# givemeone1astkiss/RNA-MPNN

Hardware: AMD Instinct MI355X
Metric: nucleotides/sec (forward), k=30 RNA graphs (higher is better)
Workload: dtype bf16; 1 GPU; C2: batch=256 RNAs, n~U[100,140], k=30, default 10-layer RNAMPNN, P=T; max_len=140, weights=closed-form deterministic init (3,536,900 params), parallelism=dp1

## Files before the change

### rna-mpnn_amd/csrc/kernels_bf16.hip

```cpp
#include "kernels_bf16.h"
#include <cstdio>
#include <cstdlib>
#include <type_traits>

#include "bf16_dev.h"
#include "graph_norm_dev.h"

__global__ void k_convert_rows_bf16(const float* __restrict__ src, int ld_src, int rows, int cols, int cols_pad,
                                    bf16_t* __restrict__ dst) {
    int id = blockIdx.x * blockDim.x + threadIdx.x;
    if (id >= rows * cols_pad) return;
    int r = id / cols_pad, c = id - r * cols_pad;
    dst[id] = c < cols ? f2bf(src[(size_t)r * ld_src + c]) : (bf16_t)0;
}
void launch_convert_rows_bf16(const float* src, int ld_src, int rows, int cols, int cols_pad, bf16_t* dst, hipStream_t s) {
    int total = rows * cols_pad;
    hipLaunchKernelGGL(k_convert_rows_bf16, dim3((total + 255) / 256), dim3(256), 0, s, src, ld_src, rows, cols, cols_pad, dst);
}

__global__ void k_build_mlp_image(const float* __restrict__ wc, int ld_wc, const float* __restrict__ w2, int ld_w2,
                                  const float* __restrict__ b2, int out_perm, bf16_t* __restrict__ img, float* __restrict__ b2p) {
    int id = blockIdx.x * blockDim.x + threadIdx.x;
    if (!w2) {
        if (id < 2 * 32 * 64 * 8) {
// ... 525 lines not shown
#undef RN_FRAG
}

static int num_cus() { return rn_num_cus(); }

void launch_mpnn_bf16(const PackInfo& pk, int k, bool do_edge, bool do_msg, const int* nbr, bf16_t* e,
                      const bf16_t* p_e, const bf16_t* q_e, const bf16_t* p_m, const bf16_t* q_m, MpnnWB we, MpnnWB wm,
                      float* agg, float* msg_out, bool edge1, const float* h_res, int reverse, hipStream_t s) {
    if (resmpnn_covers(k, edge1, msg_out != nullptr)) {
        launch_resmpnn_bf16(pk, k, do_edge, do_msg, nbr, e, p_e, q_e, p_m, q_m, we, wm, agg, h_res, reverse, s);
        return;
    }
    const int npb = k > 16 ? 1 : 32 / k;
    const int max_blocks = (pk.Nmax + npb - 1) / npb;
    int grid = (max_blocks + RN_MPNN_WAVES - 1) / RN_MPNN_WAVES;
    if (grid >= 8) grid = (grid + 7) & ~7;
    if (grid > num_cus()) grid = num_cus();
    if (grid < 1) grid = 1;
    size_t lds = RN_MPNN_LDS;
    NodeTabs tab{p_e, q_e, p_m, q_m, h_res};
    const bool smallk = k <= 16, mo = msg_out != nullptr;
#define RN_LAUNCH(E, M, S, O, E1)                                                                              \
    do {                                                                                                       \
        static DevAttr attr;                                                                                   \
        ensure_dyn_lds((const void*)k_mpnn_bf16<E, M, S, O, E1>, RN_MPNN_LDS, attr);                           \
        hipLaunchKernelGGL((k_mpnn_bf16<E, M, S, O, E1>), dim3(grid), dim3(RN_MPNN_WAVES * 64), lds, s, pk, k, nbr, e, tab, we, wm, agg, msg_out); \
    } while (0)
    if (do_edge && do_msg && edge1) { if (smallk) RN_LAUNCH(true, true, true, false, true); else RN_LAUNCH(true, true, false, false, true); }
    else if (do_edge && edge1)      { if (smallk) RN_LAUNCH(true, false, true, false, true); else RN_LAUNCH(true, false, false, false, true); }
    else if (do_edge && do_msg) { if (smallk) RN_LAUNCH(true, true, true, false, false); else RN_LAUNCH(true, true, false, false, false); }
    else if (do_edge)      { if (smallk) RN_LAUNCH(true, false, true, false, false); else RN_LAUNCH(true, false, false, false, false); }
    else if (mo)           { if (smallk) RN_LAUNCH(false, true, true, true, false); else RN_LAUNCH(false, true, false, true, false); }
    else                   { if (smallk) RN_LAUNCH(false, true, true, false, false); else RN_LAUNCH(false, true, false, false, false); }
#undef RN_LAUNCH
}

#define RN_EE_FENCE() __builtin_amdgcn_sched_barrier(0)
#ifndef EE_WAVES
#define EE_WAVES 8
#endif
template <bool SMALLK>
__global__ void __launch_bounds__(EE_WAVES * 64, EE_WAVES / 2) k_edge_embed_bf16(PackInfo pk, int k, const float* __restrict__ geomh,
        const int* __restrict__ nbr, const bf16_t* __restrict__ img_g, const float* __restrict__ b0,
        const float* __restrict__ b1p, bf16_t* __restrict__ e) {
    extern __shared__ __attribute__((aligned(16))) unsigned char smem[];
    u32x4* img = reinterpret_cast<u32x4*>(smem);
    constexpr int NFRAG = 4 * EMB_KS + 32;
    const int tid = threadIdx.x;
    float* lds_b = reinterpret_cast<float*>(smem + (size_t)NFRAG * 1024);
    if (tid < 128) lds_b[tid] = kGA * b0[tid];
    else if (tid < 256) lds_b[tid] = b1p[tid - 128];
    {
        constexpr int NT = EE_WAVES * 64, PER = (NFRAG * 64 + NT - 1) / NT;
        u32x4 t[PER];
#pragma unroll
        for (int i = 0; i < PER; ++i) t[i] = reinterpret_cast<const u32x4*>(img_g)[min(tid + i * NT, NFRAG * 64 - 1)];
#pragma unroll
        for (int i = 0; i < PER; ++i) if (tid + i * NT < NFRAG * 64) img[tid + i * NT] = t[i];
    }
    __syncthreads();
    const int ntot = pk.cu[pk.B];
    const int npb = SMALLK ? 32 / k : 1;
    const int nblocks = (ntot + npb - 1) / npb;
    const int wave = tid >> 6, lane = tid & 63, r = lane & 31, h = lane >> 5;
    const int q0 = SMALLK ? r / k : 0;
    const bool slot_ok = SMALLK ? q0 < npb : r < k;
    const int last_idx = ntot * k - 1;
    const int stride = gridDim.x * EE_WAVES;

    auto load_j = [&](int b) -> int {
        const int i = b * npb * k + r;
        const int jr = nbr[min(max(i, 0), max(last_idx, 0))];
        return (b < nblocks && slot_ok && b * npb + q0 < ntot) ? jr : -1;
    };
    f32x4 nrec[7];
    auto load_rec = [&](int j) {
        const f32x4* src = reinterpret_cast<const f32x4*>(geomh + (size_t)(j >= 0 ? j : 0) * RN_GEOMH + 32 * h);
#pragma unroll
        for (int v = 0; v < 7; ++v) nrec[v] = src[v];
    };
    int blk = blockIdx.x * EE_WAVES + wave;
    if (blk >= nblocks) return;
    int j_cur = load_j(blk), j_nxt = load_j(blk + stride);
    load_rec(j_cur);

    for (; blk < nblocks; blk += stride) {
        const int cnode = SMALLK ? min(blk * npb + q0, ntot - 1) : __builtin_amdgcn_readfirstlane(blk);
        const float* __restrict__ gc = geomh + (size_t)cnode * RN_GEOMH;
        auto catom = [&](int a, int d) { return a < 4 ? gc[3 * a + d] : gc[32 + 3 * (a - 4) + d]; };
        auto cbond = [&](int a, int d) { return a < 3 ? gc[12 + 3 * a + d] : gc[32 + 12 + 3 * (a - 3) + d]; };
        auto cnorm = [&](int a, int d) { return a < 2 ? gc[21 + 3 * a + d] : gc[32 + 21 + 3 * (a - 2) + d]; };
        float nl[28];
#pragma unroll
        for (int v = 0; v < 7; ++v) { nl[4 * v] = nrec[v][0]; nl[4 * v + 1] = nrec[v][1]; nl[4 * v + 2] = nrec[v][2]; nl[4 * v + 3] = nrec[v][3]; }
        float ft[EMB_SLOTS];
#pragma unroll
        for (int a = 0; a < 7; ++a) {
            const float ax = catom(a, 0), ay = catom(a, 1), az = catom(a, 2);
#pragma unroll
            for (int bl = 0; bl < 4; ++bl) {
                const float dx = nl[3 * bl] - ax, dy = nl[3 * bl + 1] - ay, dz = nl[3 * bl + 2] - az;
                ft[4 * a + bl] = __builtin_amdgcn_sqrtf(fmaf(dz, dz, fmaf(dy, dy, fmaf(dx, dx, kSEPS))));
            }
        }
#pragma unroll
        for (int a = 0; a < 5; ++a) {
            const float ax = cbond(a, 0), ay = cbond(a, 1), az = cbond(a, 2);
#pragma unroll
            for (int bl = 0; bl < 3; ++bl) ft[28 + 3 * a + bl] = fmaf(az, nl[12 + 3 * bl + 2], fmaf(ay, nl[12 + 3 * bl + 1], ax * nl[12 + 3 * bl]));
        }
#pragma unroll
        for (int a = 0; a < 4; ++a) {
            const float ax = cnorm(a, 0), ay = cnorm(a, 1), az = cnorm(a, 2);
#pragma unroll
            for (int bl = 0; bl < 2; ++bl) ft[43 + 2 * a + bl] = fmaf(az, nl[21 + 3 * bl + 2], fmaf(ay, nl[21 + 3 * bl + 1], ax * nl[21 + 3 * bl]));
        }
#pragma unroll
        for (int p = 51; p < EMB_SLOTS; ++p) ft[p] = 0.f;
        u32x4 xf[EMB_KS];
#pragma unroll
        for (int s = 0; s < EMB_KS; ++s)
#pragma unroll
            for (int t = 0; t < 4; ++t) xf[s][t] = p_pack2(ft[8 * s + 2 * t], ft[8 * s + 2 * t + 1]);
        RN_EE_FENCE();
        const unsigned vmask = j_cur >= 0 ? 0xffffffffu : 0u;
        load_rec(j_nxt);
        j_cur = j_nxt;
        j_nxt = load_j(blk + 2 * stride);
        RN_EE_FENCE();

        u32x4 hb[8];
#pragma unroll
        for (int mb = 0; mb < 4; ++mb) {
            f32x16 acc = init_vec16(lds_b + 32 * mb + 16 * h);
#pragma unroll
            for (int s = 0; s < EMB_KS; ++s) acc = mfma32h(img[(mb * EMB_KS + s) * 64 + lane], xf[s], acc);
#pragma unroll
            for (int t = 0; t < 4; ++t) {
                const f16x4 x = cvt_h4(acc[2 * t], acc[2 * t + 1], acc[8 + 2 * t], acc[8 + 2 * t + 1]);
                const f16x4 g = x * phi4s(x);
                hb[2 * mb][t] = __builtin_bit_cast(unsigned, lo2(g));
                hb[2 * mb + 1][t] = __builtin_bit_cast(unsigned, hi2(g));
            }
            RN_EE_FENCE();
        }
        u32x4* ewp = efrag_ptr(e, blk, lane);
#pragma unroll
        for (int ob = 0; ob < 4; ++ob) {
            f32x16 acc = init_vec16(lds_b + 128 + 32 * ob + 16 * h);
#pragma unroll
            for (int ks = 0; ks < 8; ++ks) acc = mfma32h(img[(4 * EMB_KS + ob * 8 + ks) * 64 + lane], hb[ks], acc);
#pragma unroll
            for (int sp = 0; sp < 2; ++sp) {
                u32x4 nw;
#pragma unroll
                for (int t = 0; t < 4; t += 2) {
                    const f16x4 xq = cvt_h4(acc[8 * sp + 2 * t], acc[8 * sp + 2 * t + 1], acc[8 * sp + 2 * t + 2], acc[8 * sp + 2 * t + 3]);
                    const f16x4 gq4 = xq * phi4s(xq);
                    nw[t] = __builtin_bit_cast(unsigned, lo2(gq4)) & vmask;
                    nw[t + 1] = __builtin_bit_cast(unsigned, hi2(gq4)) & vmask;
                }
                ewp[64 * (2 * ob + sp)] = nw;
            }
            RN_EE_FENCE();
        }
    }
}

void launch_edge_embed_bf16(const PackInfo& pk, int k, const float* geomh, const int* nbr, const bf16_t* img,
                            const float* b0, const float* b1p, bf16_t* e, hipStream_t s) {
    const int npb = k > 16 ? 1 : 32 / k;
    const int max_blocks = (pk.Nmax + npb - 1) / npb;
    int grid = (max_blocks + EE_WAVES - 1) / EE_WAVES;
    if (grid > 2 * num_cus()) grid = 2 * num_cus();
    if (grid < 1) grid = 1;
    size_t lds = (size_t)(4 * EMB_KS + 32) * 1024 + 1024;
    if (k > 16) hipLaunchKernelGGL(k_edge_embed_bf16<false>, dim3(grid), dim3(EE_WAVES * 64), lds, s, pk, k, geomh, nbr, img, b0, b1p, e);
    else hipLaunchKernelGGL(k_edge_embed_bf16<true>, dim3(grid), dim3(EE_WAVES * 64), lds, s, pk, k, geomh, nbr, img, b0, b1p, e);
}

#define GB_LD 72
__global__ void __launch_bounds__(256) k_gemm_bf16(const int* __restrict__ ntot_p, const float* __restrict__ X, int ldx, int K1,
        const float* __restrict__ X2, int ldx2, int K2, const bf16_t* __restrict__ W, const float* __restrict__ bias,
        int N, int act, const float* __restrict__ res, int ldres, float* __restrict__ Y, int ldy) {
    __shared__ __attribute__((aligned(16))) bf16_t As[128 * GB_LD];
    __shared__ __attribute__((aligned(16))) bf16_t Bs[128 * GB_LD];
    const int ntot = *ntot_p;
    const int row0 = blockIdx.x * 128;
    if (row0 >= ntot) return;
    const int col0 = blockIdx.y * 128;
    const int K = K1 + K2;
    const int tid = threadIdx.x, lane = tid & 63, wave = tid >> 6;
    const int r = lane & 31, h = lane >> 5;
    const int wr = wave >> 1, wc = wave & 1;
    const int srow = tid >> 1, shalf = tid & 1;

    f32x16 acc[2][2];
#pragma unroll
    for (int a = 0; a < 2; ++a)
#pragma unroll
        for (int b = 0; b < 2; ++b)
#pragma unroll
            for (int i = 0; i < 16; ++i) acc[a][b][i] = 0.f;

    f32x4 ar[8];
    u32x4 br[4];
    auto load_tile = [&](int k0) {
        const int kk = k0 + shalf * 32;
        const int row = row0 + srow;
        const bool okA = row < ntot && kk < K;
        const float* src = kk < K1 ? X + (size_t)row * ldx + kk : X2 + (size_t)row * ldx2 + (kk - K1);
#pragma unroll
        for (int v = 0; v < 8; ++v) ar[v] = okA ? *reinterpret_cast<const f32x4*>(src + 4 * v) : f32x4{0.f, 0.f, 0.f, 0.f};
        const int n = col0 + srow;
        const bool okB = n < N && kk < K;
        const u32x4* wsrc = reinterpret_cast<const u32x4*>(W + (size_t)n * K + kk);
#pragma unroll
        for (int v = 0; v < 4; ++v) br[v] = okB ? wsrc[v] : u32x4{0u, 0u, 0u, 0u};
    };
    auto store_tile = [&]() {
        u32x4* da = reinterpret_cast<u32x4*>(As + srow * GB_LD + shalf * 32);
#pragma unroll
        for (int v = 0; v < 4; ++v) {
            u32x4 w;
            w[0] = pack2(ar[2 * v][0], ar[2 * v][1]); w[1] = pack2(ar[2 * v][2], ar[2 * v][3]);
            w[2] = pack2(ar[2 * v + 1][0], ar[2 * v + 1][1]); w[3] = pack2(ar[2 * v + 1][2], ar[2 * v + 1][3]);
            da[v] = w;
        }
        u32x4* db = reinterpret_cast<u32x4*>(Bs + srow * GB_LD + shalf * 32);
#pragma unroll
        for (int v = 0; v < 4; ++v) db[v] = br[v];
    };

    load_tile(0);
    for (int k0 = 0; k0 < K; k0 += 64) {
        __syncthreads();
        store_tile();
        __syncthreads();
        if (k0 + 64 < K) load_tile(k0 + 64);
#pragma unroll
        for (int ks = 0; ks < 4; ++ks) {
            u32x4 af[2], bfm[2];
#pragma unroll
            for (int t = 0; t < 2; ++t) {
                af[t] = *reinterpret_cast<const u32x4*>(As + (64 * wr + 32 * t + r) * GB_LD + 16 * ks + 8 * h);
                bfm[t] = *reinterpret_cast<const u32x4*>(Bs + (64 * wc + 32 * t + r) * GB_LD + 16 * ks + 8 * h);
            }
#pragma unroll
            for (int a = 0; a < 2; ++a)
#pragma unroll
                for (int b = 0; b < 2; ++b) acc[a][b] = mfma32(af[a], bfm[b], acc[a][b]);
        }
    }
    const bool has_res = res != nullptr;
#pragma unroll
    for (int b = 0; b < 2; ++b) {
        const int col = col0 + 64 * wc + 32 * b + r;
        const bool colok = col < N;
        const int cc = colok ? col : 0;
        const float bv = bias ? bias[cc] : 0.f;
#pragma unroll
        for (int a = 0; a < 2; ++a) {
            const int rbase = row0 + 64 * wr + 32 * a + 4 * h;
            float v[16], rv[16];
            if (has_res) {
#pragma unroll
                for (int i = 0; i < 16; ++i) {
                    const int row = rbase + (i & 3) + 8 * (i >> 2);
                    rv[i] = res[(size_t)(row < ntot ? row : ntot - 1) * ldres + cc];
                }
            }
#pragma unroll
            for (int i = 0; i < 16; ++i) v[i] = acc[a][b][i] + bv;
            if (act == 1) {
#pragma unroll
                for (int i = 0; i < 16; ++i) v[i] = gelu_erf(v[i]);
            }
            if (has_res) {
#pragma unroll
                for (int i = 0; i < 16; ++i) v[i] += rv[i];
            }
#pragma unroll
            for (int i = 0; i < 16; ++i) {
                const int row = rbase + (i & 3) + 8 * (i >> 2);
                if (colok && row < ntot) Y[(size_t)row * ldy + col] = v[i];
            }
        }
    }
}

void launch_gemm_bf16(const int* ntot, int mmax, const float* X, int ldx, int K1, const float* X2, int ldx2, int K2,
                      const bf16_t* W, const float* bias, int N, int act, const float* res, int ldres,
                      float* Y, int ldy, hipStream_t s) {
    dim3 grid((mmax + 127) / 128, (N + 127) / 128);
    hipLaunchKernelGGL(k_gemm_bf16, grid, dim3(256), 0, s, ntot, X, ldx, K1, X2, ldx2, K2, W, bias, N, act, res, ldres, Y, ldy);
}

struct ChainW {
    const bf16_t* img;
    const float* bias[5];
};

#define CH_RING 4
#if !defined(RN_EXPERIMENTS) && (defined(CH_EXP_NODMA) || defined(CH_EXP_NOGELU) || defined(CH_EXP_NOLDS) || defined(CH_EXP_NOBAR) || defined(CH_GRANULES1))
#error "k_ffn_chain ablations need -DRN_EXPERIMENTS"
#endif
#ifndef CH_GELU
#define CH_GELU 1
#endif
__device__ __forceinline__ void chain_issue(const u32x4* __restrict__ img, u32x4* ring, int c, int tid) {
    const u32x4* src = img + (size_t)c * 2048 + tid;
    u32x4* dst = ring + (c % CH_RING) * 2048 + (tid & ~63);
#pragma unroll
    for (int i = 0; i < 8; ++i)
        __builtin_amdgcn_global_load_lds((const __attribute__((address_space(1))) void*)(src + i * 256),
                                         (__attribute__((address_space(3))) void*)(dst + i * 256), 16, 0, 0);
}
__device__ __forceinline__ void chain_issue_piece(const u32x4* __restrict__ img, u32x4* ring, int c, int tid, int i) {
#ifdef CH_EXP_NODMA
    return;
#endif
    const u32x4* src = img + (size_t)c * 2048 + tid + i * 256;
    u32x4* dst = ring + (c % CH_RING) * 2048 + (tid & ~63) + i * 256;
    __builtin_amdgcn_global_load_lds((const __attribute__((address_space(1))) void*)src,
                                     (__attribute__((address_space(3))) void*)dst, 16, 0, 0);
}
__device__ __forceinline__ void chain_wait(int chunks_after) {
    if (chunks_after >= 2) asm volatile("s_waitcnt vmcnt(16)" ::: "memory");
    else if (chunks_after == 1) asm volatile("s_waitcnt vmcnt(8)" ::: "memory");
    else asm volatile("s_waitcnt vmcnt(0)" ::: "memory");
#ifndef CH_EXP_NOBAR
    __builtin_amdgcn_s_barrier();
#endif
}

template <int NKS, int NOB, int C0, int NCH_T, bool LAST>
__device__ __forceinline__ void chain_layer(const u32x4* __restrict__ img, u32x4* ring, int tid, int lane, int h,
                                            const u32x4 (&in)[32], u32x4 (&out)[32], const float* bias_lds,
                                            float* __restrict__ yrow, int n_valid, bool row_ok) {
    constexpr int OPC = 32 / NKS, NCH = NOB / OPC;
    f32x16 accA, accB;
    auto granule = [&](const f32x16& acc, auto obc, auto tc) {
        constexpr int ob = decltype(obc)::value, t = decltype(tc)::value;
#ifdef CH_EXP_NOGELU
        if constexpr (!LAST) { out[2 * ob][t] = __float_as_uint(acc[2 * t]); out[2 * ob + 1][t] = __float_as_uint(acc[8 + 2 * t]); return; }
#endif
        if constexpr (!LAST) {
#if CH_GELU == 2
            const f16x4 g = cvt_h4(gelu_fast(acc[2 * t]), gelu_fast(acc[2 * t + 1]), gelu_fast(acc[8 + 2 * t]), gelu_fast(acc[8 + 2 * t + 1]));
#else
            const f16x4 x = cvt_h4(acc[2 * t], acc[2 * t + 1], acc[8 + 2 * t], acc[8 + 2 * t + 1]);
#if CH_GELU == 1
            const f16x4 g = x * phi5n(x);
#else
            const f16x4 g = x * phi4(x);
#endif
#endif
            out[2 * ob][t] = __builtin_bit_cast(unsigned, lo2(g));
            out[2 * ob + 1][t] = __builtin_bit_cast(unsigned, hi2(g));
        } else if (row_ok) {
            const int c0 = 32 * ob + 16 * h + 4 * t;
            if (c0 < n_valid) *reinterpret_cast<f32x4*>(yrow + c0) = f32x4{acc[4 * t], acc[4 * t + 1], acc[4 * t + 2], acc[4 * t + 3]};
        }
    };
    static_for<NCH>([&](auto chc) {
        constexpr int ch = decltype(chc)::value, c = C0 + ch;
        chain_wait(NCH_T - 1 - c < 2 ? NCH_T - 1 - c : 2);
        const u32x4* buf = ring + (c % CH_RING) * 2048 + lane;
        u32x4 fr[8];
#pragma unroll
        for (int m = 0; m < 8; ++m) fr[m] = buf[m * 64];
        static_for<OPC>([&](auto oc) {
            constexpr int o = decltype(oc)::value, ob = ch * OPC + o;
            f32x16& acc = (ob & 1) ? accB : accA;
            f32x16& prev = (ob & 1) ? accA : accB;
            acc = init_vec16(bias_lds + 32 * ob + 16 * h);
            static_for<NKS>([&](auto ksc) {
                constexpr int ks = decltype(ksc)::value, m = o * NKS + ks;
                acc = mfma32h(fr[m & 7], in[ks], acc);
#ifndef CH_EXP_NOLDS
                if constexpr (m + 8 < 32) fr[m & 7] = buf[(m + 8) * 64];
#endif
                if constexpr (c + 3 < NCH_T && (m & 3) == 1) chain_issue_piece(img, ring, c + 3, tid, m >> 2);
                __builtin_amdgcn_sched_barrier(0);
                if constexpr (ob > 0) {
#ifndef CH_GRANULES1
                    if constexpr (NKS >= 4) {
                        if constexpr ((ks + 1) % (NKS / 4) == 0)
                            granule(prev, std::integral_constant<int, (ob > 0 ? ob - 1 : 0)>{}, std::integral_constant<int, (ks + 1) / (NKS / 4) - 1>{});
                    } else {
                        granule(prev, std::integral_constant<int, (ob > 0 ? ob - 1 : 0)>{}, std::integral_constant<int, (2 * ks) & 3>{});
                        granule(prev, std::integral_constant<int, (ob > 0 ? ob - 1 : 0)>{}, std::integral_constant<int, (2 * ks + 1) & 3>{});
                    }
#else
                    if constexpr (ks == (NKS >= 2 ? NKS / 2 - 1 : 0))
                        static_for<4>([&](auto tc) { granule(prev, std::integral_constant<int, (ob > 0 ? ob - 1 : 0)>{}, tc); });
#endif
                    __builtin_amdgcn_sched_barrier(0);
                }
            });
        });
    });
    static_for<4>([&](auto tc) { granule(((NOB - 1) & 1) ? accB : accA, std::integral_constant<int, NOB - 1>{}, tc); });
    __builtin_amdgcn_sched_barrier(0);
}

template <int K0, int H, int NH, int NOUT>
__global__ void __launch_bounds__(256, 1) k_ffn_chain(const int* __restrict__ ntot_p, const float* __restrict__ X, int ldx,
        const float* __restrict__ X2, int ldx2, ChainW w, float* __restrict__ Y, int ldy, int n_valid) {
    extern __shared__ __attribute__((aligned(16))) unsigned char smem[];
    u32x4* ring = reinterpret_cast<u32x4*>(smem);
    float* bias_lds = reinterpret_cast<float*>(smem + CH_RING * 32768);
    const int ntot = *ntot_p;
    const int row_blk = blockIdx.x * 128;
    if (row_blk >= ntot) return;
    const int tid = threadIdx.x, lane = tid & 63, wave = tid >> 6, r = lane & 31, h = lane >> 5;
    const int row = row_blk + 32 * wave + r;
    const bool row_ok = row < ntot;
    constexpr int HK = H / 16, HB = H / 32, OB = NOUT / 32;
    constexpr int NCH0 = HB * (K0 / 16) / 32, NCHH = HB * HK / 32, NCHL = OB * HK / 32, NCH_T = NCH0 + NH * NCHH + NCHL;
    {
        constexpr int NBL = ((NH + 1) * H + NOUT + 255) / 256;
        float bv[NBL];
#pragma unroll
        for (int t = 0; t < NBL; ++t) {
            const int idx = tid + 256 * t;
            const int l = idx / H < NH + 1 ? idx / H : NH + 1, i = idx - l * H;
            bv[t] = (idx < (NH + 1) * H + NOUT) ? (CH_GELU == 1 && l < NH + 1 ? kGAn : 1.f) * w.bias[l][i] : 0.f;
        }
#pragma unroll
        for (int t = 0; t < NBL; ++t) if (tid + 256 * t < (NH + 1) * H + NOUT) bias_lds[tid + 256 * t] = bv[t];
    }
    u32x4 a[32], b[32];
    {
        const int rr = row_ok ? row : ntot - 1;
        f32x4 v0[K0 / 16], v1[K0 / 16];
#pragma unroll
        for (int s = 0; s < K0 / 16; ++s) {
            const int kk = 16 * s + 8 * h;
            const float* src = (K0 > 128 && kk >= 128) ? X2 + (size_t)rr * ldx2 + (kk - 128) : X + (size_t)rr * ldx + kk;
            v0[s] = *reinterpret_cast<const f32x4*>(src);
            v1[s] = *reinterpret_cast<const f32x4*>(src + 4);
        }
#pragma unroll
        for (int s = 0; s < K0 / 16; ++s)
            a[s] = u32x4{p_pack2(v0[s][0], v0[s][1]), p_pack2(v0[s][2], v0[s][3]), p_pack2(v1[s][0], v1[s][1]), p_pack2(v1[s][2], v1[s][3])};
    }
    __syncthreads();
    const u32x4* img = reinterpret_cast<const u32x4*>(w.img);
    chain_issue(img, ring, 0, tid);
    if (NCH_T > 1) chain_issue(img, ring, 1, tid);
    if (NCH_T > 2) chain_issue(img, ring, 2, tid);
    float* yrow = Y + (size_t)row * ldy;
    chain_layer<K0 / 16, HB, 0, NCH_T, false>(img, ring, tid, lane, h, a, b, bias_lds, yrow, n_valid, row_ok);
    if (NH == 0) {
        chain_layer<HK, OB, NCH0, NCH_T, true>(img, ring, tid, lane, h, b, a, bias_lds + H, yrow, n_valid, row_ok);
    } else if (NH == 1) {
        chain_layer<HK, HB, NCH0, NCH_T, false>(img, ring, tid, lane, h, b, a, bias_lds + H, yrow, n_valid, row_ok);
        chain_layer<HK, OB, NCH0 + NCHH, NCH_T, true>(img, ring, tid, lane, h, a, b, bias_lds + 2 * H, yrow, n_valid, row_ok);
    } else {
        chain_layer<HK, HB, NCH0, NCH_T, false>(img, ring, tid, lane, h, b, a, bias_lds + H, yrow, n_valid, row_ok);
        chain_layer<HK, HB, NCH0 + NCHH, NCH_T, false>(img, ring, tid, lane, h, a, b, bias_lds + 2 * H, yrow, n_valid, row_ok);
        chain_layer<HK, OB, NCH0 + 2 * NCHH, NCH_T, true>(img, ring, tid, lane, h, b, a, bias_lds + 3 * H, yrow, n_valid, row_ok);
    }
}

__global__ void k_build_chain_image(const float* __restrict__ wraw, int K_real, int K, int N, int n_real, int first, float wscale,
                                    bf16_t* __restrict__ dst) {
    int id = blockIdx.x * blockDim.x + threadIdx.x;
    int nks = K / 16;
    if (id >= (N / 32) * nks * 64 * 8) return;
    int j = id & 7, lane = (id >> 3) & 63, f = id >> 9;
    int ob = f / nks, ks = f % nks, r = lane & 31, h = lane >> 5;
    int row = ch_nat(ob, r);
    int col = first ? 16 * ks + 8 * h + j : 32 * (ks >> 1) + 16 * h + 8 * (ks & 1) + j;
    const float wv = (row < n_real && col < K_real) ? wraw[(size_t)row * K_real + col] : 0.f;
    dst[id] = __builtin_bit_cast(bf16_t, (_Float16)(wscale * wv));
}
void launch_build_chain_image(const float* wraw, int K_real, int K, int N, int n_real, int position, bf16_t* dst, hipStream_t s) {
    int total = (N / 32) * (K / 16) * 512;
    const float wscale = CH_GELU == 1 ? (position == 0 ? kGAn : position == 2 ? kGAni : 1.f) : 1.f;
    hipLaunchKernelGGL(k_build_chain_image, dim3((total + 255) / 256), dim3(256), 0, s, wraw, K_real, K, N, n_real, position == 0 ? 1 : 0, wscale, dst);
}

int launch_ffn_chain(const int* ntot, int mmax, const float* X, int ldx, const float* X2, int ldx2, int K0, int H, int NH,
                     int NOUT, const bf16_t* img, const float* const* bias, float* Y, int ldy, int n_valid, hipStream_t s) {
    ChainW w;
    w.img = img;
    for (int i = 0; i < 5; ++i) w.bias[i] = i < NH + 2 ? bias[i] : nullptr;
    dim3 grid((mmax + 127) / 128);
    const size_t lds = CH_RING * 32768 + (size_t)((NH + 1) * H + NOUT) * sizeof(float);
#define RN_CHAIN(k0, hh, nh, no) \
    if (K0 == k0 && H == hh && NH == nh && NOUT == no) { \
        static DevAttr attr; \
        ensure_dyn_lds((const void*)k_ffn_chain<k0, hh, nh, no>, lds, attr); \
        hipLaunchKernelGGL((k_ffn_chain<k0, hh, nh, no>), grid, dim3(256), lds, s, ntot, X, ldx, X2, ldx2, w, Y, ldy, n_valid); return 0; }
    RN_CHAIN(128, 512, 2, 128)
    RN_CHAIN(32, 512, 2, 128)
    RN_CHAIN(256, 512, 0, 32)
#undef RN_CHAIN
    return 1;
}

__global__ void __launch_bounds__(256) k_gn_coef(PackInfo pk, const float* __restrict__ x, const float* __restrict__ scale,
        const float* __restrict__ shift, int t_tot, float* __restrict__ coef) {
    __shared__ float4 red[4][8];
    const int b = blockIdx.x, cg = blockIdx.y;
    const int n = pk.len[b];
    if (n <= 0) return;
    const size_t base = (size_t)pk.cu[b] * RN_D + 32 * cg;
    const int cq = threadIdx.x & 7, g = threadIdx.x >> 3;
    const int wave = threadIdx.x >> 6, lane = threadIdx.x & 63;
    const float4* xb = reinterpret_cast<const float4*>(x + base) + cq;
    auto block_sum = [&](float4 s) -> float4 {
#pragma unroll
        for (int o = 8; o < 64; o <<= 1) {
            s.x += __shfl_xor(s.x, o, 64); s.y += __shfl_xor(s.y, o, 64); s.z += __shfl_xor(s.z, o, 64); s.w += __shfl_xor(s.w, o, 64);
        }
        __syncthreads();
        if (lane < 8) red[wave][lane] = s;
        __syncthreads();
        float4 t = red[0][cq];
#pragma unroll
        for (int w = 1; w < 4; ++w) { const float4 u = red[w][cq]; t.x += u.x; t.y += u.y; t.z += u.z; t.w += u.w; }
        return t;
    };
    const float fn = (float)n;
    float4 mu, Q;
    auto stats = [&](const auto& rows) {
        const float4 S = block_sum(rows.sum());
        mu = make_float4(S.x / fn, S.y / fn, S.z / fn, S.w / fn);
        Q = block_sum(rows.sqdev(mu));
    };
    if (n <= 160) stats(GnRows<32, 5>(xb, g, n));
    else if (n <= 256) stats(GnRows<32, 8>(xb, g, n));
    else stats(GnRows<32, 0>(xb, g, n));
    if (threadIdx.x < 8) {
        const float4 sc = reinterpret_cast<const float4*>(scale + 32 * cg)[cq], sh = reinterpret_cast<const float4*>(shift + 32 * cg)[cq];
        float4 a, bb;
        gn_affine(Q.x, mu.x, n, t_tot, sc.x, sh.x, a.x, bb.x); gn_affine(Q.y, mu.y, n, t_tot, sc.y, sh.y, a.y, bb.y);
        gn_affine(Q.z, mu.z, n, t_tot, sc.z, sh.z, a.z, bb.z); gn_affine(Q.w, mu.w, n, t_tot, sc.w, sh.w, a.w, bb.w);
        float* cb = coef + (size_t)b * 256 + 32 * cg + 4 * cq;
        *reinterpret_cast<float4*>(cb) = a;
        *reinterpret_cast<float4*>(cb + 128) = bb;
    }
}

typedef NodeJob PqJob;

__device__ __forceinline__ void node_load_row(const float* __restrict__ x, int row, int h, f32x4 (&vx)[8][2]) {
#pragma unroll
    for (int s = 0; s < 8; ++s) {
        const int c0 = 16 * s + 8 * h;
        vx[s][0] = *reinterpret_cast<const f32x4*>(x + (size_t)row * RN_D + c0);
        vx[s][1] = *reinterpret_cast<const f32x4*>(x + (size_t)row * RN_D + c0 + 4);
    }
}
template <int NJOBS, int NT>
__device__ __forceinline__ void node_stage(u32x4* img, float* lds_bias, const PqJob& j0, const PqJob& j1, int tid) {
    __builtin_amdgcn_sched_barrier(0);
    stage_image_dma<NT>(img, reinterpret_cast<const u32x4*>(j0.img), tid);
    if (NJOBS > 1) stage_image_dma<NT>(img + 4096, reinterpret_cast<const u32x4*>(j1.img), tid);
    __builtin_amdgcn_sched_barrier(0);
    if (tid < 128) lds_bias[tid] = j0.bias[tid];
    else if (NJOBS > 1 && tid < 256) lds_bias[tid] = j1.bias[tid - 128];
}
__device__ __forceinline__ void node_affine(const float* ab, int h, f32x4 (&vx)[8][2]) {
#pragma unroll
    for (int s = 0; s < 8; ++s) {
        const int c0 = 16 * s + 8 * h;
        const f32x4 ca0 = *reinterpret_cast<const f32x4*>(ab + c0), ca1 = *reinterpret_cast<const f32x4*>(ab + c0 + 4);
        const f32x4 cb0 = *reinterpret_cast<const f32x4*>(ab + 128 + c0), cb1 = *reinterpret_cast<const f32x4*>(ab + 128 + c0 + 4);
        vx[s][0] = vx[s][0] * ca0 + cb0; vx[s][1] = vx[s][1] * ca1 + cb1;
    }
}
__device__ __forceinline__ void node_pack_store(const f32x4 (&vx)[8][2], u32x4 (&xf)[8], float* __restrict__ h_out, int row, bool ok, int h) {
#pragma unroll
    for (int s = 0; s < 8; ++s) {
        const f32x4 v0 = vx[s][0], v1 = vx[s][1];
        xf[s] = u32x4{p_pack2(v0[0], v0[1]), p_pack2(v0[2], v0[3]), p_pack2(v1[0], v1[1]), p_pack2(v1[2], v1[3])};
    }
    __builtin_amdgcn_sched_barrier(0);
    dma_landed();
    __builtin_amdgcn_sched_barrier(0);
    if (ok && h_out) {
#pragma unroll
        for (int s = 0; s < 8; ++s) {
            const int c0 = 16 * s + 8 * h;
            *reinterpret_cast<f32x4*>(h_out + (size_t)row * RN_D + c0) = vx[s][0];
            *reinterpret_cast<f32x4*>(h_out + (size_t)row * RN_D + c0 + 4) = vx[s][1];
        }
    }
}
template <int NJOBS>
__device__ __forceinline__ void node_project(const u32x4* img, const float* lds_bias, const u32x4 (&xf)[8], const PqJob& j0, const PqJob& j1,
                                             int row, bool ok, int lane, int h) {
#pragma unroll
    for (int jb = 0; jb < NJOBS; ++jb) {
        const PqJob& jbq = jb == 0 ? j0 : j1;
        const u32x4* im = img + jb * 4096;
#pragma unroll
        for (int ob = 0; ob < 8; ++ob) {
            f32x16 acc;
            if (ob < 4) acc = init_vec16(lds_bias + jb * 128 + 32 * ob + 16 * h);
            else {
#pragma unroll
                for (int i = 0; i < 16; ++i) acc[i] = 0.f;
            }
#pragma unroll
            for (int ks = 0; ks < 8; ++ks) acc = mfma32h(im[(ob * 8 + ks) * 64 + lane], xf[ks], acc);
            if (ok) {
                bf16_t* row_p = (ob < 4 ? jbq.p : jbq.q) + (size_t)row * RN_D + 32 * (ob & 3);
                const bool efr = ob < 4 && jbq.p_efrag;
                u32x4* d0 = reinterpret_cast<u32x4*>(row_p + (efr ? 8 * h : 16 * h));
                u32x4* d1 = reinterpret_cast<u32x4*>(row_p + (efr ? 16 + 8 * h : 16 * h + 8));
                *d0 = u32x4{p_pack2(acc[0], acc[1]), p_pack2(acc[2], acc[3]), p_pack2(acc[4], acc[5]), p_pack2(acc[6], acc[7])};
                *d1 = u32x4{p_pack2(acc[8], acc[9]), p_pack2(acc[10], acc[11]), p_pack2(acc[12], acc[13]), p_pack2(acc[14], acc[15])};
            }
            __builtin_amdgcn_sched_barrier(0);
        }
    }
    asm volatile("s_waitcnt vmcnt(0)" ::: "memory");
}

template <int NJOBS>
__global__ void __launch_bounds__(256) __attribute__((amdgpu_waves_per_eu(2, 3))) k_node_update(PackInfo pk, const float* __restrict__ x, const float* __restrict__ coef,
        float* __restrict__ h_out, PqJob j0, PqJob j1) {
    extern __shared__ __attribute__((aligned(16))) unsigned char smem[];
    u32x4* img = reinterpret_cast<u32x4*>(smem);
    float* lds_bias = reinterpret_cast<float*>(smem + NJOBS * 65536);
    const int ntot = pk.cu[pk.B];
    const int row_blk = blockIdx.x * 128;
    if (row_blk >= ntot) return;
    const int tid = threadIdx.x, lane = tid & 63, wave = tid >> 6, r = lane & 31, h = lane >> 5;
    const int row = row_blk + 32 * wave + r;
    const bool ok = row < ntot;
    const int rr = ok ? row : 0;
    const float* cf = coef + (size_t)pk.node_b[rr] * 256;
    f32x4 vx[8][2];
    node_load_row(x, rr, h, vx);
    node_stage<NJOBS, 256>(img, lds_bias, j0, j1, tid);
    if (coef) node_affine(cf, h, vx);
    u32x4 xf[8];
    node_pack_store(vx, xf, h_out, row, ok, h);
    __syncthreads();
    node_project<NJOBS>(img, lds_bias, xf, j0, j1, row, ok, lane, h);
}

template <int CTRL, int ROW_MASK>
__device__ __forceinline__ float dpp_f32(float v) {
    return __builtin_bit_cast(float, __builtin_amdgcn_update_dpp(0, __builtin_bit_cast(int, v), CTRL, ROW_MASK, 0xf, ROW_MASK == 0xf));
}
__device__ __forceinline__ float half_wave_sum2(float a, float b) {
    asm volatile("s_nop 1\n\tv_permlane16_swap_b32 %0, %1\n\ts_nop 1" : "+v"(a), "+v"(b));
    float v = a + b;
    v += dpp_f32<0xB1, 0xf>(v);
    v += dpp_f32<0x4E, 0xf>(v);
    v += dpp_f32<0x141, 0xf>(v);
    v += dpp_f32<0x140, 0xf>(v);
    return v;
}
template <int NJOBS, int NB>
__global__ void __launch_bounds__(NB * 64) k_node_update_rna(PackInfo pk, const float* __restrict__ x, const float* __restrict__ scale,
        const float* __restrict__ shift, int t_tot, float* __restrict__ h_out, PqJob j0, PqJob j1) {
    extern __shared__ __attribute__((aligned(16))) unsigned char smem[];
    u32x4* img = reinterpret_cast<u32x4*>(smem);
    float* lds_bias = reinterpret_cast<float*>(smem + NJOBS * 65536);
    float* lds_part = lds_bias + 256;
    float* lds_mean = lds_part + NB * 128;
    float* lds_ab = lds_mean + 128;
    const int b = blockIdx.x;
    const int n = pk.len[b];
    if (n <= 0) return;
    const int base = pk.cu[b];
    const int tid = threadIdx.x, lane = tid & 63, wave = tid >> 6, r = lane & 31, h = lane >> 5;
    const int rb = wave;
    const int lrow = 32 * rb + r;
    const bool ok = lrow < n;
    const int row = base + (ok ? lrow : 0);
    f32x4 vx[8][2];
    node_load_row(x, row, h, vx);
    node_stage<NJOBS, NB * 64>(img, lds_bias, j0, j1, tid);
    float sc_c = 0.f, sh_c = 0.f;
    if (tid < 128) { sc_c = scale[tid]; sh_c = shift[tid]; }
    const int nwb = (n + 31) >> 5;
    auto reduce_rows = [&](auto&& value) {
#pragma unroll
        for (int s = 0; s < 4; ++s) {
            f32x4 t0, t1;
#pragma unroll
            for (int i = 0; i < 4; ++i) { t0[i] = half_wave_sum2(value(s, 0, i), value(s + 4, 0, i)); t1[i] = half_wave_sum2(value(s, 1, i), value(s + 4, 1, i)); }
            if ((r & 15) == 0) {
                const int sb = s + (r >> 4) * 4;
                *reinterpret_cast<f32x4*>(lds_part + rb * 128 + 16 * sb + 8 * h) = t0;
                *reinterpret_cast<f32x4*>(lds_part + rb * 128 + 16 * sb + 8 * h + 4) = t1;
            }
        }
    };
    auto combine = [&]() -> float {
        float t = lds_part[tid];
        for (int w = 1; w < nwb; ++w) t += lds_part[w * 128 + tid];
        return t;
    };
    reduce_rows([&](int s, int p, int i) { return ok ? vx[s][p][i] : 0.f; });
    __syncthreads();
    float mean_c = 0.f;
    if (tid < 128) { mean_c = combine() / (float)n; lds_mean[tid] = mean_c; }
    __syncthreads();
    f32x4 mu[8][2];
#pragma unroll
    for (int s = 0; s < 8; ++s) {
        mu[s][0] = *reinterpret_cast<const f32x4*>(lds_mean + 16 * s + 8 * h);
        mu[s][1] = *reinterpret_cast<const f32x4*>(lds_mean + 16 * s + 8 * h + 4);
    }
    reduce_rows([&](int s, int p, int i) { const float d = vx[s][p][i] - mu[s][p][i]; return ok ? d * d : 0.f; });
    __syncthreads();
    if (tid < 128) {
        float a, bb;
        gn_affine(combine(), mean_c, n, t_tot, sc_c, sh_c, a, bb);
        lds_ab[tid] = a;
        lds_ab[128 + tid] = bb;
    }
    __syncthreads();
    node_affine(lds_ab, h, vx);
    u32x4 xf[8];
    node_pack_store(vx, xf, h_out, row, ok, h);
    __syncthreads();
    if (rb >= nwb) return;
    node_project<NJOBS>(img, lds_bias, xf, j0, j1, row, ok, lane, h);
}

__global__ void k_build_pq_image(const float* __restrict__ w0, const float* __restrict__ b1, int efrag, bf16_t* __restrict__ dst,
                                 float* __restrict__ b1p) {
    int id = blockIdx.x * blockDim.x + threadIdx.x;
    if (id >= 8 * 8 * 64 * 8) return;
    int j = id & 7, lane = (id >> 3) & 63, f = id >> 9, ob = f >> 3, ks = f & 7, r = lane & 31, h = lane >> 5;
    int row = (efrag && ob < 4) ? ch_efrag(ob, r) : ch_nat(ob & 3, r), col = (ob < 4 ? 0 : 128) + 16 * ks + 8 * h + j;
    dst[id] = __builtin_bit_cast(bf16_t, (_Float16)(kGA * w0[(size_t)row * 384 + col]));
    if (id < 128) {
        int ob2 = id >> 5, m = id & 31, hh = (m >> 2) & 1, i = (m & 3) + 4 * (m >> 3);
        b1p[32 * ob2 + 16 * hh + i] = kGA * b1[efrag ? ch_efrag(ob2, m) : ch_nat(ob2, m)];
    }
}
void launch_build_pq_image(const float* w0, const float* b1, int efrag, bf16_t* dst, float* b1p, hipStream_t s) {
    hipLaunchKernelGGL(k_build_pq_image, dim3(8 * 8 * 64 * 8 / 256), dim3(256), 0, s, w0, b1, efrag, dst, b1p);
}

void launch_node_update(const PackInfo& pk, const float* x, const float* scale, const float* shift, int t_tot, float* coef,
                        float* h_out, int njobs, const NodeJob& job0, const NodeJob& job1, hipStream_t s) {
    const PqJob j0 = job0, j1 = njobs > 1 ? job1 : NodeJob{};
    if (scale && pk.T >= 48 && pk.T <= 256 && !ab_switch("RNAMPNN_NODE_UPDATE_TWO_LAUNCH")) {
#define NU_RNA(J, NBK)                                                                                                          \
        do {                                                                                                                    \
            static DevAttr attr;                                                                                                \
            constexpr size_t lds = (size_t)(J) * 65536 + 1024 + (NBK) * 512 + 3 * 512;                                          \
            ensure_dyn_lds((const void*)k_node_update_rna<J, NBK>, lds, attr);                                                  \
            hipLaunchKernelGGL((k_node_update_rna<J, NBK>), dim3(pk.B), dim3((NBK) * 64), lds, s, pk, x, scale, shift, t_tot, h_out, j0, j1); \
        } while (0)
        if (njobs == 1) { if (pk.T <= 128) NU_RNA(1, 4); else if (pk.T <= 160) NU_RNA(1, 5); else NU_RNA(1, 8); }
        else { if (pk.T <= 128) NU_RNA(2, 4); else if (pk.T <= 160) NU_RNA(2, 5); else NU_RNA(2, 8); }
#undef NU_RNA
        return;
    }
    if (scale) hipLaunchKernelGGL(k_gn_coef, dim3(pk.B, 4), dim3(256), 0, s, pk, x, scale, shift, t_tot, coef);
    dim3 grid((pk.Nmax + 127) / 128);
    static DevAttr attr1, attr2;
// ... 337 lines not shown
```

Measured before the change: 14.37 million nucleotides/s.

## Hand-schedule FFN chain: explicit LDS reads, rotated DMA, spread GELU epilogue

Reworks the fused FFN chain kernel's inner schedule. It issues LDS fragment reads via inline ds_read_b128 with fine-grained lgkmcnt waits, precomputes scalar/vector DMA addresses and rotates the DMA piece order by block index, and splits the GELU epilogue into 64 micro-ops spread over MFMA slots that carry no DMA issue. The aim is to hide LDS latency and epilogue ALU work behind matrix instructions and to reduce address arithmetic and DRAM channel contention. It adds heavy inline-asm scheduling constraints that may limit compiler freedom and removes the CH_GRANULES1 ablation.

```diff
diff --git a/rna-mpnn_amd/csrc/kernels_bf16.hip b/rna-mpnn_amd/csrc/kernels_bf16.hip
--- a/rna-mpnn_amd/csrc/kernels_bf16.hip
+++ b/rna-mpnn_amd/csrc/kernels_bf16.hip
@@ -851,28 +851,33 @@
 };
 
 #define CH_RING 4
-#if !defined(RN_EXPERIMENTS) && (defined(CH_EXP_NODMA) || defined(CH_EXP_NOGELU) || defined(CH_EXP_NOLDS) || defined(CH_EXP_NOBAR) || defined(CH_GRANULES1))
+#if !defined(RN_EXPERIMENTS) && (defined(CH_EXP_NODMA) || defined(CH_EXP_NOGELU) || defined(CH_EXP_NOLDS) || defined(CH_EXP_NOBAR))
 #error "k_ffn_chain ablations need -DRN_EXPERIMENTS"
 #endif
 #ifndef CH_GELU
 #define CH_GELU 1
 #endif
-__device__ __forceinline__ void chain_issue(const u32x4* __restrict__ img, u32x4* ring, int c, int tid) {
-    const u32x4* src = img + (size_t)c * 2048 + tid;
-    u32x4* dst = ring + (c % CH_RING) * 2048 + (tid & ~63);
-#pragma unroll
-    for (int i = 0; i < 8; ++i)
-        __builtin_amdgcn_global_load_lds((const __attribute__((address_space(1))) void*)(src + i * 256),
-                                         (__attribute__((address_space(3))) void*)(dst + i * 256), 16, 0, 0);
-}
-__device__ __forceinline__ void chain_issue_piece(const u32x4* __restrict__ img, u32x4* ring, int c, int tid, int i) {
+#define CH_GLOBAL __attribute__((address_space(1)))
+#define CH_LOCAL __attribute__((address_space(3)))
+struct ChainDma {
+    const CH_GLOBAL char* src;
+    CH_LOCAL char* dst;
+    unsigned l16;
+    unsigned rot;
+};
+__device__ __forceinline__ void chain_issue_piece(ChainDma& d, int c, int i) {
 #ifdef CH_EXP_NODMA
     return;
 #endif
-    const u32x4* src = img + (size_t)c * 2048 + tid + i * 256;
-    u32x4* dst = ring + (c % CH_RING) * 2048 + (tid & ~63) + i * 256;
-    __builtin_amdgcn_global_load_lds((const __attribute__((address_space(1))) void*)src,
-                                     (__attribute__((address_space(3))) void*)dst, 16, 0, 0);
+    const unsigned ib = ((unsigned)(i + d.rot) & 7u) * 4096u;
+    const CH_GLOBAL char* g = d.src + (size_t)c * 32768 + ib;
+    asm("" : "+s"(g));
+    asm volatile("" : "+v"(d.l16));
+    __builtin_amdgcn_global_load_lds((const CH_GLOBAL void*)(g + d.l16), (CH_LOCAL void*)(d.dst + (c % CH_RING) * 32768 + ib), 16, 0, 0);
+}
+__device__ __forceinline__ void chain_issue(ChainDma& d, int c) {
+#pragma unroll
+    for (int i = 0; i < 8; ++i) chain_issue_piece(d, c, i);
 }
 __device__ __forceinline__ void chain_wait(int chunks_after) {
     if (chunks_after >= 2) asm volatile("s_waitcnt vmcnt(16)" ::: "memory");
@@ -882,13 +887,51 @@
     __builtin_amdgcn_s_barrier();
 #endif
 }
+__device__ __forceinline__ void chain_frag_read(u32x4& fr, unsigned lds_addr, int byte_off) {
+    asm volatile("ds_read_b128 %0, %1 offset:%2" : "=v"(fr) : "v"(lds_addr), "n"(byte_off));
+}
+template <int N>
+__device__ __forceinline__ void chain_frag_wait(u32x4& fr) {
+    asm volatile("s_waitcnt lgkmcnt(%1)" : "+v"(fr) : "n"(N));
+}
+
+__host__ __device__ constexpr bool ch_dma_gap(int c, int nch_t, int m) { return c + 3 < nch_t && (m & 3) == 1; }
+__host__ __device__ constexpr int ch_free_gaps(int c, int nch_t, int m0, int n) {
+    int f = 0;
+    for (int m = m0; m < m0 + n; ++m) f += ch_dma_gap(c, nch_t, m) ? 0 : 1;
+    return f;
+}
+__host__ __device__ constexpr int ch_epi_mid2(int j) { const int jj = j & 15; return 40 * (j >> 4) + (jj < 2 ? 6 * jj + 3 : 2 * (4 + jj) + 1); }
+__host__ __device__ constexpr int ch_epi_first(int fi, int nfree) {
+    int j = 0;
+    while (j < 64 && ch_epi_mid2(j) * nfree / 160 < fi) ++j;
+    return j;
+}
 
 template <int NKS, int NOB, int C0, int NCH_T, bool LAST>
-__device__ __forceinline__ void chain_layer(const u32x4* __restrict__ img, u32x4* ring, int tid, int lane, int h,
+__device__ __forceinline__ void chain_layer(ChainDma& dma, unsigned ring_lane, int h,
                                             const u32x4 (&in)[32], u32x4 (&out)[32], const float* bias_lds,
                                             float* __restrict__ yrow, int n_valid, bool row_ok) {
     constexpr int OPC = 32 / NKS, NCH = NOB / OPC;
+#if CH_GELU == 1 && !defined(CH_EXP_NOGELU)
+    constexpr bool SPREAD = !LAST;
+#else
+    constexpr bool SPREAD = false;
+#endif
     f32x16 accA, accB;
+    f16x2 ex[2], es[2], eq[2];
+    auto epi_op = [&](const f32x16& acc, auto obc, auto jc) {
+        constexpr int ob = decltype(obc)::value, j = decltype(jc)::value, t = j >> 4, u = (j & 15) >> 1, hf = j & 1;
+        f16x2 &x = ex[hf], &s = es[hf], &q = eq[hf];
+        if constexpr (u == 0) x = cvt_h2(acc[8 * hf + 2 * t], acc[8 * hf + 2 * t + 1]);
+        else if constexpr (u == 1) s = clamp01h(x * x);
+        else if constexpr (u == 2) q = __builtin_elementwise_fma(s, h2(RN_QN4), h2(RN_QN3));
+        else if constexpr (u == 3) q = __builtin_elementwise_fma(q, s, h2(RN_QN2));
+        else if constexpr (u == 4) q = __builtin_elementwise_fma(q, s, h2(RN_QN1));
+        else if constexpr (u == 5) q = __builtin_elementwise_fma(q, s, h2(RN_QN0));
+        else if constexpr (u == 6) q = clamp01h(__builtin_elementwise_fma(x, q, h2(0.5f)));
+        else out[2 * ob + hf][t] = __builtin_bit_cast(unsigned, x * q);
+    };
     auto granule = [&](const f32x16& acc, auto obc, auto tc) {
         constexpr int ob = decltype(obc)::value, t = decltype(tc)::value;
 #ifdef CH_EXP_NOGELU
@@ -915,42 +958,57 @@
     static_for<NCH>([&](auto chc) {
         constexpr int ch = decltype(chc)::value, c = C0 + ch;
         chain_wait(NCH_T - 1 - c < 2 ? NCH_T - 1 - c : 2);
-        const u32x4* buf = ring + (c % CH_RING) * 2048 + lane;
+        __builtin_amdgcn_sched_barrier(0);
+        const unsigned buf = ring_lane + (c % CH_RING) * 32768;
         u32x4 fr[8];
 #pragma unroll
-        for (int m = 0; m < 8; ++m) fr[m] = buf[m * 64];
+        for (int m = 0; m < 8; ++m) chain_frag_read(fr[m], buf, m * 1024);
+#ifndef CH_EXP_NOLDS
+        chain_frag_wait<7>(fr[0]);
+#else
+#pragma unroll
+        for (int m = 0; m < 8; ++m) chain_frag_wait<0>(fr[m]);
+#endif
         static_for<OPC>([&](auto oc) {
             constexpr int o = decltype(oc)::value, ob = ch * OPC + o;
+            constexpr int NFREE = ch_free_gaps(c, NCH_T, o * NKS, NKS);
+            static_assert(NFREE > 0, "a block without a free gap");
             f32x16& acc = (ob & 1) ? accB : accA;
             f32x16& prev = (ob & 1) ? accA : accB;
             acc = init_vec16(bias_lds + 32 * ob + 16 * h);
             static_for<NKS>([&](auto ksc) {
                 constexpr int ks = decltype(ksc)::value, m = o * NKS + ks;
                 acc = mfma32h(fr[m & 7], in[ks], acc);
+                __builtin_amdgcn_sched_barrier(0);
 #ifndef CH_EXP_NOLDS
-                if constexpr (m + 8 < 32) fr[m & 7] = buf[(m + 8) * 64];
+                if constexpr (m + 8 < 32) chain_frag_read(fr[m & 7], buf, (m + 8) * 1024);
+                if constexpr (m + 1 < 32) chain_frag_wait<(30 - m < 7 ? 30 - m : 7)>(fr[(m + 1) & 7]);
 #endif
-                if constexpr (c + 3 < NCH_T && (m & 3) == 1) chain_issue_piece(img, ring, c + 3, tid, m >> 2);
+                if constexpr (ch_dma_gap(c, NCH_T, m)) chain_issue_piece(dma, c + 3, m >> 2);
                 __builtin_amdgcn_sched_barrier(0);
                 if constexpr (ob > 0) {
-#ifndef CH_GRANULES1
-                    if constexpr (NKS >= 4) {
+                    constexpr int obp = ob > 0 ? ob - 1 : 0;
+                    if constexpr (SPREAD) {
+                        if constexpr (!ch_dma_gap(c, NCH_T, m)) {
+                            constexpr int fi = ch_free_gaps(c, NCH_T, o * NKS, ks), j0 = ch_epi_first(fi, NFREE), j1 = ch_epi_first(fi + 1, NFREE);
+                            static_for<j1 - j0>([&](auto jc) { epi_op(prev, std::integral_constant<int, obp>{}, std::integral_constant<int, j0 + decltype(jc)::value>{}); });
+                        }
+                    } else if constexpr (NKS >= 4) {
                         if constexpr ((ks + 1) % (NKS / 4) == 0)
-                            granule(prev, std::integral_constant<int, (ob > 0 ? ob - 1 : 0)>{}, std::integral_constant<int, (ks + 1) / (NKS / 4) - 1>{});
+                            granule(prev, std::integral_constant<int, obp>{}, std::integral_constant<int, (ks + 1) / (NKS / 4) - 1>{});
                     } else {
-                        granule(prev, std::integral_constant<int, (ob > 0 ? ob - 1 : 0)>{}, std::integral_constant<int, (2 * ks) & 3>{});
-                        granule(prev, std::integral_constant<int, (ob > 0 ? ob - 1 : 0)>{}, std::integral_constant<int, (2 * ks + 1) & 3>{});
+                        granule(prev, std::integral_constant<int, obp>{}, std::integral_constant<int, (2 * ks) & 3>{});
+                        granule(prev, std::integral_constant<int, obp>{}, std::integral_constant<int, (2 * ks + 1) & 3>{});
                     }
-#else
-                    if constexpr (ks == (NKS >= 2 ? NKS / 2 - 1 : 0))
-                        static_for<4>([&](auto tc) { granule(prev, std::integral_constant<int, (ob > 0 ? ob - 1 : 0)>{}, tc); });
-#endif
                     __builtin_amdgcn_sched_barrier(0);
                 }
             });
         });
     });
-    static_for<4>([&](auto tc) { granule(((NOB - 1) & 1) ? accB : accA, std::integral_constant<int, NOB - 1>{}, tc); });
+    if constexpr (SPREAD)
+        static_for<64>([&](auto jc) { epi_op(((NOB - 1) & 1) ? accB : accA, std::integral_constant<int, NOB - 1>{}, jc); });
+    else
+        static_for<4>([&](auto tc) { granule(((NOB - 1) & 1) ? accB : accA, std::integral_constant<int, NOB - 1>{}, tc); });
     __builtin_amdgcn_sched_barrier(0);
 }
 
@@ -996,21 +1054,23 @@
             a[s] = u32x4{p_pack2(v0[s][0], v0[s][1]), p_pack2(v0[s][2], v0[s][3]), p_pack2(v1[s][0], v1[s][1]), p_pack2(v1[s][2], v1[s][3])};
     }
     __syncthreads();
-    const u32x4* img = reinterpret_cast<const u32x4*>(w.img);
-    chain_issue(img, ring, 0, tid);
-    if (NCH_T > 1) chain_issue(img, ring, 1, tid);
-    if (NCH_T > 2) chain_issue(img, ring, 2, tid);
+    const int wave_u = __builtin_amdgcn_readfirstlane(wave);
+    ChainDma dma{(const CH_GLOBAL char*)w.img + wave_u * 1024, (CH_LOCAL char*)ring + wave_u * 1024, (unsigned)lane * 16u, blockIdx.x};
+    const unsigned ring_lane = (unsigned)(size_t)(CH_LOCAL char*)ring + (unsigned)lane * 16u;
+    chain_issue(dma, 0);
+    if (NCH_T > 1) chain_issue(dma, 1);
+    if (NCH_T > 2) chain_issue(dma, 2);
     float* yrow = Y + (size_t)row * ldy;
-    chain_layer<K0 / 16, HB, 0, NCH_T, false>(img, ring, tid, lane, h, a, b, bias_lds, yrow, n_valid, row_ok);
+    chain_layer<K0 / 16, HB, 0, NCH_T, false>(dma, ring_lane, h, a, b, bias_lds, yrow, n_valid, row_ok);
     if (NH == 0) {
-        chain_layer<HK, OB, NCH0, NCH_T, true>(img, ring, tid, lane, h, b, a, bias_lds + H, yrow, n_valid, row_ok);
+        chain_layer<HK, OB, NCH0, NCH_T, true>(dma, ring_lane, h, b, a, bias_lds + H, yrow, n_valid, row_ok);
     } else if (NH == 1) {
-        chain_layer<HK, HB, NCH0, NCH_T, false>(img, ring, tid, lane, h, b, a, bias_lds + H, yrow, n_valid, row_ok);
-        chain_layer<HK, OB, NCH0 + NCHH, NCH_T, true>(img, ring, tid, lane, h, a, b, bias_lds + 2 * H, yrow, n_valid, row_ok);
+        chain_layer<HK, HB, NCH0, NCH_T, false>(dma, ring_lane, h, b, a, bias_lds + H, yrow, n_valid, row_ok);
+        chain_layer<HK, OB, NCH0 + NCHH, NCH_T, true>(dma, ring_lane, h, a, b, bias_lds + 2 * H, yrow, n_valid, row_ok);
     } else {
-        chain_layer<HK, HB, NCH0, NCH_T, false>(img, ring, tid, lane, h, b, a, bias_lds + H, yrow, n_valid, row_ok);
-        chain_layer<HK, HB, NCH0 + NCHH, NCH_T, false>(img, ring, tid, lane, h, a, b, bias_lds + 2 * H, yrow, n_valid, row_ok);
-        chain_layer<HK, OB, NCH0 + 2 * NCHH, NCH_T, true>(img, ring, tid, lane, h, b, a, bias_lds + 3 * H, yrow, n_valid, row_ok);
+        chain_layer<HK, HB, NCH0, NCH_T, false>(dma, ring_lane, h, b, a, bias_lds + H, yrow, n_valid, row_ok);
+        chain_layer<HK, HB, NCH0 + NCHH, NCH_T, false>(dma, ring_lane, h, a, b, bias_lds + 2 * H, yrow, n_valid, row_ok);
+        chain_layer<HK, OB, NCH0 + 2 * NCHH, NCH_T, true>(dma, ring_lane, h, b, a, bias_lds + 3 * H, yrow, n_valid, row_ok);
     }
 }
 
```

Result: no change. 14.49 million nucleotides/s (median of 6 runs) (+0.8%).
